# kentril0/WaterSurfaceRendering

Measured on AMD Instinct MI355X. Metric: ocean frames/s (ComputeWaves, 7 fields -> displacement + normal map), higher is better.
Workload: dtype f32; 1 GPU; 2048x2048 tile, FULL7, reference default parameters; tile_size=2048, tiles_per_rank=1, pipeline_depth=3, seed=1592590336, parallelism=tiles sharded 1 process per GPU x1, no data-path collective

## Files before the change

watersurfacerendering_amd/csrc/ocean_kernels.h:

```cpp
#pragma once
#include <hip/hip_runtime.h>
#include <hip/hip_fp16.h>
#include <stdint.h>
#include <type_traits>
#include "fft_engine.h"

namespace ocean {

typedef float ocean_f4 __attribute__((ext_vector_type(4)));
__device__ __forceinline__ void store_nt(float4* p, float4 v)
{
    ocean_f4 t = {v.x, v.y, v.z, v.w};
    __builtin_nontemporal_store(t, reinterpret_cast<ocean_f4*>(p));
}
__device__ __forceinline__ void store_f2_sc1(float2* base, unsigned byte_off, float2 v)
{
    typedef float f2v __attribute__((ext_vector_type(2)));
    const f2v t = {v.x, v.y};
    asm volatile("global_store_dwordx2 %0, %1, %2 sc1" ::"v"(byte_off), "v"(t), "s"(base) : "memory");
}
template <bool NTS> __device__ __forceinline__ void store_map(float4* base, unsigned texel, float4 v)
{
    float4* p = reinterpret_cast<float4*>(reinterpret_cast<char*>(base) + (texel * 16u));
    if constexpr (NTS) store_nt(p, v);
// ... 227 lines not shown
            float4 ha[PB];
            float2 hb0[PB], hb1[PB], wv[PB];
#pragma unroll
            for (int u = 0; u < PB; ++u) {
                const int it = tid + (ub + u) * T;
                const int c = COLS == 1 ? 0 : it / PAIRS, n = 2 * (COLS == 1 ? it : it % PAIRS);
                if (!GUARD || it < ITEMS) zpass_load_pair<N, H16, W16, ZNT>(a, tile, nb + c, n, h16s, base, ha[u], hb0[u], hb1[u], wv[u]);
            }
#pragma unroll
            for (int u = 0; u < PB; ++u) {
                const int it = tid + (ub + u) * T;
                const int c = COLS == 1 ? 0 : it / PAIRS, n = 2 * (COLS == 1 ? it : it % PAIRS);
                if (!GUARD || it < ITEMS) {
                    float a0, b0, a1, b1;
                    animate_with_mirror(make_float2(ha[u].x, ha[u].y), hb0[u], wv[u].x, t, a0, b0);
                    animate_with_mirror(make_float2(ha[u].z, ha[u].w), hb1[u], wv[u].y, t, a1, b1);
                    *reinterpret_cast<float2*>((c ? sp + N : sp) + n) = col0 ? make_float2(a0, a1) : make_float2(0.5f * (a0 + b0), 0.5f * (a1 + b1));
                    if constexpr (KZ_LDS) *reinterpret_cast<float2*>(kzt + n) = *reinterpret_cast<const float2*>(k1 + n);
                    if (n == 0) raw[c] = 0.5f * (a0 - b0);
                }
            }
        }
    });
}

template <int N> struct Half {
    static constexpr int NU = N / 2 + 1;
    static constexpr int NUP = (N / 2 + 16) & ~15;
    static constexpr size_t Z_GROUP = (size_t)NU * 2 * NUP;
    static constexpr size_t Z_TILE = 3 * Z_GROUP;
    static constexpr size_t ZH_TILE = (size_t)NU * NUP;
    static constexpr size_t HRAW_TILE = (size_t)NUP * N;
    template <bool Z16> static constexpr int zb() { return Z16 ? 16 : 8; }
    static_assert(NUP % 16 == 0, "row blocks");
    template <bool Z16> static __device__ __forceinline__ unsigned zidx(int nb, int side, int q)
    {
        constexpr int ZB = zb<Z16>();
        return (unsigned)(((q / ZB) * 2 + side) * (NU * ZB) + nb * ZB + (q % ZB));
    }
    template <bool Z16> static __device__ __forceinline__ unsigned zhidx(int nb, int q)
    {
        constexpr int ZB = zb<Z16>() > 8 ? zb<Z16>() : 8;
        return (unsigned)((q / ZB) * (NU * ZB) + nb * ZB + (q % ZB));
    }
};
__device__ __forceinline__ unsigned hraw_index(int n, int p, int u) { return (unsigned)(u * n + p); }

__device__ __forceinline__ int xcd_swizzle(int id, int n)
{
    const int q = n / 8, r = n % 8, x = id % 8;
    return (x < r ? x * (q + 1) : r * (q + 1) + (x - r) * q) + id / 8;
}

template <int N, int T, class P, int ZC, bool Z16> struct ZStore {
    using HF = Half<N>;
    using LS = LastStage<N, ZC, T, P>;
    static constexpr int S = LS::STRIDE, NU = HF::NU;
    static constexpr int ZB = HF::template zb<Z16>(), ZBH = ZB > 8 ? ZB : 8;
    static constexpr bool FAST = S >= ZBH && S % ZBH == 0 && (N / 2) % S == 0 && !(Z16 && ZC == 4);
    int b0[LS::IT], b1[LS::IT], bh[LS::IT];
    static __device__ __forceinline__ int reg(int v) { asm("" : "+v"(v)); return v; }
    __device__ __forceinline__ void init(int tid, int nb, bool two_columns = false)
    {
        if constexpr (FAST) {
#pragma unroll
            for (int u = 0; u < LS::IT; ++u) {
                const int w = tid + u * T;
                int c = 0, j = 0;
                if (!LS::GUARD || w < LS::ITEMS) LS::map(w, c, j);
                const int col = nb + (two_columns ? c : 0);
                b0[u] = (j / ZB) * (2 * NU * ZB) + (j % ZB) + col * ZB;
                const int cj = (j + ZB - 1) / ZB, rj = (ZB - j % ZB) % ZB;
                b1[u] = NU * ZB + col * ZB + rj - cj * (2 * NU * ZB);
                bh[u] = (j / ZBH) * (NU * ZBH) + (j % ZBH) + col * ZBH;
            }
        }
    }
    __device__ __forceinline__ unsigned pos(int col, int p, int u, int i) const
    {
        if constexpr (!FAST) return p <= N / 2 ? HF::template zidx<Z16>(col, 0, p) : HF::template zidx<Z16>(col, 1, N - p);
        else {
            const int lo = i * S;
            if (lo < N / 2) return (unsigned)(reg(b0[u]) + (lo / ZB) * (2 * NU * ZB));
            const int far = reg(b1[u]) + ((N - lo) / ZB) * (2 * NU * ZB);
            if (lo > N / 2) return (unsigned)far;
            return (unsigned)(far - (p == N / 2 ? NU * ZB : 0));
        }
    }
    __device__ __forceinline__ bool keeps(int p, int i) const
    {
        if constexpr (!FAST) return p <= N / 2;
        else return i * S < N / 2 || (i * S == N / 2 && p == N / 2);
    }
    __device__ __forceinline__ unsigned hpos(int col, int p, int u, int i) const
    {
        if constexpr (!FAST) return HF::template zhidx<Z16>(col, p);
        else return (unsigned)(reg(bh[u]) + ((i * S) / ZBH) * (NU * ZBH));
    }
};


template <int N> constexpr int zpass_columns() { return (N == 512 || N == 256) ? 4 : 2; }
template <int N> constexpr bool zpass_has_width2() { return zpass_columns<N>() == 2 && N >= 1024 && N <= 2048; }

template <int FIRST, int SLOTS>
__device__ __forceinline__ c32 zpass_input_slot(int c, float kx, float kx2, float kz, float sv, float tx, float tz, float tc,
                                                float choppy, float full7, bool jac, float g3)
{
#pragma clang fp contract(off)
    static_assert(FIRST + SLOTS <= 4 && (SLOTS == 1 || SLOTS == 4 || (SLOTS == 2 && FIRST % 2 == 0)), "one pair, {pair 0, pair 1}, {pair 2, pair 3} or all four");
    constexpr bool ODD_PAIRS = FIRST < 2, EVEN_PAIRS = FIRST + SLOTS > 2;
    const int pair = SLOTS == 1 ? FIRST : FIRST + c;
    const float d = __builtin_fmaf(kz, kz, kx2);
    const float inv = d > 1e-10f ? rsqrtf(d) : 0.0f;
    if (ODD_PAIRS && (!EVEN_PAIRS || pair < 2)) {
        const float f = (pair ? -1.0f : inv) * choppy;
        return make_float2(kz * f * tz, -kx * f * tx);
    }
    const float g = full7 * inv * sv;
    return pair == 2 ? make_float2(kx2 * g, kz * kz * g) : make_float2(sv, jac ? g3 * (kx * kz * inv * tc) : 0.0f);
}
template <int PAIR>
__device__ __forceinline__ c32 zpass_input(float kx, float kx2, float kz, float sv, float tx, float tz, float tc, bool jac, float g3)
{
#pragma clang fp contract(off)
    const float d = __builtin_fmaf(kz, kz, kx2);
    const float inv = d > 1e-10f ? rsqrtf(d) : 0.0f;
    if constexpr (PAIR == 0) { const float f = inv; return make_float2(kz * f * tz, -kx * f * tx); }
    else if constexpr (PAIR == 1) { const float f = -1.0f; return make_float2(kz * f * tz, -kx * f * tx); }
    else if constexpr (PAIR == 2) { const float g = inv * sv; return make_float2(kx2 * g, (kz * kz) * g); }
    else return make_float2(sv, jac ? g3 * (kx * kz * inv * tc) : 0.0f);
}
template <int N, bool COL0>
__device__ __forceinline__ void zpass_fetch(const float* sp, float sm0, int e, float& sv, float& tx, float& tz, float& tc)
{
    if constexpr (COL0) {
        const float g1 = sp[e], g2 = sp[(N - e) & (N - 1)];
        sv = 0.5f * (g1 + g2);
        tx = 0.5f * (g1 - g2);
        tz = (e == 0) ? tx : sv;
        tc = (e == 0) ? sv : tx;
    } else {
        sv = sp[e];
        tx = sv;
        tz = (e == 0) ? sm0 : sv;
        tc = tz;
    }
}
template <int N, bool Z16> struct ZOut {
    float su = 1.0f, sk = 1.0f, s3 = 1.0f, g3 = 1.0f;
    float2* __restrict__ zt;
    float2* __restrict__ z3;
// ... 156 lines not shown
        }
        if (blk == LAST) { one_column(N / 2); return; }
        one_column(0);
        __syncthreads();
        one_column(1);
    } else {
        one_column(xcd_swizzle(bx, gx));
    }
}

template <int N, int T, class P = Plan<N>, bool ZNT = false, bool Z16 = false, int ZW = 1, bool FAST = true>
__global__ void __launch_bounds__(T, zpass_min_waves<N>()) k_zpass(const FrameArgs a)
{
    extern __shared__ __attribute__((aligned(16))) unsigned char smem[];
    zpass_body<N, T, P, ZNT, Z16, ZW, FAST>(a, smem, (int)blockIdx.x, (int)gridDim.x);
}

__device__ __forceinline__ void start_ramp_wait(int ramp, unsigned idx, unsigned count)
{
    if (ramp > 0) {
        const unsigned until = idx * (unsigned)ramp / count;
        const unsigned long long t0 = wall_clock64();
        while ((unsigned)(wall_clock64() - t0) < until) __builtin_amdgcn_s_sleep(4);
    }
}

#ifdef OCEAN_CLOCKPROBE
static __device__ unsigned long long* g_clockprobe = nullptr;
constexpr unsigned CLOCKPROBE_LAUNCHES = 4096, CLOCKPROBE_WGS = 1032;
struct ClockProbe {
    unsigned long long* p;
    unsigned long long c0, r0;
    __device__ explicit ClockProbe(unsigned launch) : p(nullptr), c0(0), r0(0)
    {
        if (threadIdx.x == 0 && g_clockprobe && blockIdx.y == 0 && blockIdx.x < CLOCKPROBE_WGS) {
            p = g_clockprobe + 4 * ((size_t)(launch % CLOCKPROBE_LAUNCHES) * CLOCKPROBE_WGS + blockIdx.x);
            c0 = __builtin_amdgcn_s_memtime();
            r0 = __builtin_amdgcn_s_memrealtime();
        }
    }
    __device__ void end()
    {
        if (p) {
            const unsigned long long c1 = __builtin_amdgcn_s_memtime(), r1 = __builtin_amdgcn_s_memrealtime();
            unsigned hwid, xcc;
            asm volatile("s_getreg_b32 %0, hwreg(HW_REG_HW_ID)" : "=s"(hwid));
            asm volatile("s_getreg_b32 %0, hwreg(HW_REG_XCC_ID)" : "=s"(xcc));
            p[0] = r0; p[1] = r1; p[2] = c1 - c0; p[3] = (unsigned long long)xcc | ((unsigned long long)hwid << 32);
        }
    }
};
#endif

template <int N, int T, class P, bool COL0, bool ZNT, bool Z16, bool ZWT = false>
__device__ __forceinline__ void zpass_single_transforms(const FrameArgs& a, c32* fbuf, const float* sp, const float (&kzr)[P::r[0]],
                                                        TwiddleRegs<N, 1, T, P>& twr, float kx, float sm0, int tid, int tile, int nb)
{
    using HF = Half<N>;
    static_assert(FirstStage<N, 1, T, P>::IT == 1, "one first-stage butterfly per thread");
    const float kx2 = kx * kx;
    [[maybe_unused]] float su = 1.0f, sk = 1.0f, s3 = 1.0f;
    float g3 = 1.0f;
    if constexpr (Z16) { const float4 zs = a.zscale[2 * tile]; su = zs.x; sk = zs.y; s3 = a.zscale[2 * tile + 1].x; }
    if (a.mode == 3) g3 = a.zscale[2 * tile + 1].y;
    constexpr size_t ES = Z16 ? 4 : 8;
    float2* __restrict__ zt = reinterpret_cast<float2*>(reinterpret_cast<char*>(a.z) + (size_t)tile * HF::Z_TILE * ES);
    float2* __restrict__ z3 = reinterpret_cast<float2*>(reinterpret_cast<char*>(a.z3) + (size_t)tile * HF::Z_GROUP * ES);
    float2* __restrict__ zh = reinterpret_cast<float2*>(reinterpret_cast<char*>(a.zh) + (size_t)tile * HF::ZH_TILE * ES);
    const bool jac = a.mode == 3;
    ZStore<N, T, P, 1, Z16> zo;
    zo.init(tid, nb);
    auto fetch = [&](int e, float& sv, float& tx, float& tz, float& tc) {
        if constexpr (COL0) {
            const float g1 = sp[e], g2 = sp[(N - e) & (N - 1)];
            sv = 0.5f * (g1 + g2);
            tx = 0.5f * (g1 - g2);
            tz = (e == 0) ? tx : sv;
            tc = (e == 0) ? sv : tx;
        } else {
            sv = sp[e];
            tx = sv;
            tz = (e == 0) ? sm0 : sv;
            tc = tz;
        }
    };
    if (a.mode != 2) {
        if (a.zmask & 1) {
            auto in = [&](int e, int, int, int i) -> c32 {
                float sv, tx, tz, tc; fetch(e, sv, tx, tz, tc);
                return zpass_input<0>(kx, kx2, kzr[i], sv, tx, tz, tc, false, 1.0f);
            };
            auto out = [&](int p, int, c32 v, int u, int i) { store_z<ZNT, Z16, ZWT>(zt, zo.pos(nb, p, u, i), v, su); };
            batch_fft<N, 1, T, P>(fbuf, twr, tid, in, out);
        }
        if (a.zmask & 2) {
            auto in = [&](int e, int, int, int i) -> c32 {
                float sv, tx, tz, tc; fetch(e, sv, tx, tz, tc);
                return zpass_input<1>(kx, kx2, kzr[i], sv, tx, tz, tc, false, 1.0f);
            };
            auto out = [&](int p, int, c32 v, int u, int i) { store_z<ZNT, Z16, ZWT>(zt, (unsigned)HF::Z_GROUP + zo.pos(nb, p, u, i), v, sk); };
            batch_fft<N, 1, T, P>(fbuf, twr, tid, in, out);
        }
    }
    if ((a.mode == 0 || a.mode == 3) && (a.zmask & 4)) {
        auto in = [&](int e, int, int, int i) -> c32 {
            float sv, tx, tz, tc; fetch(e, sv, tx, tz, tc);
            return zpass_input<2>(kx, kx2, kzr[i], sv, tx, tz, tc, false, 1.0f);
        };
        auto out = [&](int p, int, c32 v, int u, int i) { store_z<ZNT, Z16, ZWT>(zt, 2u * (unsigned)HF::Z_GROUP + zo.pos(nb, p, u, i), v, sk); };
        batch_fft<N, 1, T, P>(fbuf, twr, tid, in, out);
    }
    if (a.zmask & 8) {
        auto in = [&](int e, int, int, int i) -> c32 {
            float sv, tx, tz, tc; fetch(e, sv, tx, tz, tc);
            if (!jac) return make_float2(sv, 0.0f);
            return zpass_input<3>(kx, kx2, kzr[i], sv, tx, tz, tc, true, g3);
        };
        auto out = [&](int p, int, c32 v, int u, int i) {
            if (jac) store_z<ZNT, Z16, ZWT>(z3, zo.pos(nb, p, u, i), v, s3);
            else if (zo.keeps(p, i)) store_z<ZNT, Z16, ZWT>(zh, zo.hpos(nb, p, u, i), v, su);
        };
        batch_fft<N, 1, T, P>(fbuf, twr, tid, in, out);
    }
}

template <int N> constexpr size_t zpass_c1_lds_bytes() { return sizeof(c32) * fft_lds_elems<N, 1>() + sizeof(float) * N; }
template <int N, int T, bool FAST> constexpr int zpass_c1_min_waves() { return T == N / 16 ? 3 : (FAST ? 6 : 5); }
template <int N, int T, class P, bool ZNT = false, bool Z16 = false, bool FAST = true, bool ZWT = false>
__global__ void __launch_bounds__(T, (zpass_c1_min_waves<N, T, FAST>())) k_zpass_c1(const FrameArgs a)
{
    extern __shared__ __attribute__((aligned(16))) unsigned char smem[];
    c32* fbuf = reinterpret_cast<c32*>(smem);
    float* sp = reinterpret_cast<float*>(fbuf + fft_lds_elems<N, 1>());
    float* raw = reinterpret_cast<float*>(fbuf);
    const int tid = threadIdx.x;
    const int tile = blockIdx.y;
#ifdef OCEAN_CLOCKPROBE
    ClockProbe clock_probe_(a.frame_seq);
#endif
    start_ramp_wait(a.start_ramp, blockIdx.x, gridDim.x);
    TwiddleRegs<N, 1, T, P> twr;
    twr.load(a.tw, tid);
#ifdef OCEAN_DEVELOPER
    const int bxr = (blockIdx.x % 8 == 0 || a.xcd_rot == 0) ? (int)blockIdx.x : (int)(blockIdx.x / 8 * 8 + 1 + (blockIdx.x % 8 - 1 + a.xcd_rot) % 7);
    const int nb = xcd_swizzle(bxr, N / 2 + 1);
#else
    const int nb = xcd_swizzle((int)blockIdx.x, N / 2 + 1);
#endif
    const float t = a.t + (a.toff ? a.toff[tile] : 0.0f);
    const float* __restrict__ k1 = a.k1d + (size_t)tile * N;
    const bool col0 = (nb == 0);
    const float h16s = a.h0h ? a.h0_inv_scale[tile] : 1.0f;
    const float base = a.omega_q ? a.base_freq[tile] : 0.0f;
    spectrum_form<FAST>(a, [&](auto h16, auto w16) {
        constexpr bool H16 = decltype(h16)::value, W16 = decltype(w16)::value;
        constexpr int PAIRS = N / 2;
        constexpr int P1 = (PAIRS + T - 1) / T;
        constexpr int PB = P1 > 4 ? 4 : P1;
        static_assert(P1 % PB == 0 && PAIRS % T == 0, "phase-1 batches");
#pragma unroll 1
        for (int ub = 0; ub < P1; ub += PB) {
            float4 ha[PB];
            float2 hb0[PB], hb1[PB], wv[PB];
#pragma unroll
            for (int u = 0; u < PB; ++u)
                zpass_load_pair<N, H16, W16, ZNT>(a, tile, nb, 2 * (tid + (ub + u) * T), h16s, base, ha[u], hb0[u], hb1[u], wv[u]);
#pragma unroll
            for (int u = 0; u < PB; ++u) {
                const int n = 2 * (tid + (ub + u) * T);
                float a0, b0, a1, b1;
                animate_with_mirror(make_float2(ha[u].x, ha[u].y), hb0[u], wv[u].x, t, a0, b0);
                animate_with_mirror(make_float2(ha[u].z, ha[u].w), hb1[u], wv[u].y, t, a1, b1);
                *reinterpret_cast<float2*>(sp + n) = col0 ? make_float2(a0, a1) : make_float2(0.5f * (a0 + b0), 0.5f * (a1 + b1));
                if (n == 0) raw[0] = 0.5f * (a0 - b0);
            }
        }
    });
    if (blockIdx.x == 0 && tid == 0 && (a.zmask & 8)) {
        a.minmax[2 * tile + 0] = float_key(3.402823466e+38f);
        a.minmax[2 * tile + 1] = float_key(1.175494351e-38f);
        a.hdone[tile] = 0u;
    }
    float kzr[P::r[0]];
#pragma unroll
    for (int i = 0; i < P::r[0]; ++i) kzr[i] = k1[tid + i * (N / P::r[0])];
    __syncthreads();
    const float sm0 = raw[0];
    static_assert(!ZWT || (!ZNT && !Z16), "write-through is a policy of the plain fp32 intermediates");
    if (col0) zpass_single_transforms<N, T, P, true, ZNT, Z16, ZWT>(a, fbuf, sp, kzr, twr, k1[nb], sm0, tid, tile, nb);
    else zpass_single_transforms<N, T, P, false, ZNT, Z16, ZWT>(a, fbuf, sp, kzr, twr, k1[nb], sm0, tid, tile, nb);
#ifdef OCEAN_CLOCKPROBE
    clock_probe_.end();
#endif
}
template <int N> constexpr bool zpass_has_c1() { return N >= 1024; }
template <int N> inline bool zpass_c1_pays(bool nt_inter, unsigned tiles)
{
    if (N == 4096) return true;
    if (nt_inter) return false;
    return N == 2048 || tiles >= 2;
}

template <int N, int T> constexpr int zpass_blocks_per_cu()
{
    constexpr int by_lds = (int)(163840 / (sizeof(c32) * fft_lds_elems<N, zpass_columns<N>()>() + sizeof(float) * 2 * N));
    constexpr int by_threads = 2048 / T;
    constexpr int by_regs = (zpass_min_waves<N>() * 4 * 64) / T;
    constexpr int m = by_lds < by_threads ? by_lds : by_threads;
    return (by_regs >= 1 && by_regs < m) ? by_regs : (m < 1 ? 1 : m);
}

template <int N, int ZW = 1> constexpr size_t zpass_lds_bytes()
{
    return sizeof(c32) * fft_lds_elems<N, zpass_columns<N>()>() + sizeof(float) * 2 * N;
}


__device__ __forceinline__ void store_wt(float* p, float v) { __hip_atomic_store(p, v, __ATOMIC_RELAXED, __HIP_MEMORY_SCOPE_AGENT); }
__device__ __forceinline__ float load_wt(const float* p) { return __hip_atomic_load(p, __ATOMIC_RELAXED, __HIP_MEMORY_SCOPE_AGENT); }
__device__ __forceinline__ unsigned load_wt(const unsigned* p) { return __hip_atomic_load(p, __ATOMIC_RELAXED, __HIP_MEMORY_SCOPE_AGENT); }
__device__ __forceinline__ void wait_counter(const unsigned* ctr, unsigned target, int tid, int poll_sleep = 0, unsigned* fault = nullptr)
{
    if (tid == 0) {
#ifdef OCEAN_FAULT_INJECT
        target += 1u;
#endif
        const unsigned long long t0 = wall_clock64();
        bool ok;
        while (!(ok = load_wt(ctr) >= target) && (wall_clock64() - t0) < 2000000ull) {
            if (poll_sleep <= 0) __builtin_amdgcn_s_sleep(2);
            else for (int k = 0; k < poll_sleep; ++k) __builtin_amdgcn_s_sleep(127);
        }
        if (!ok && fault) *fault = 1u;
    }
    __syncthreads();
}

__device__ __forceinline__ void wait_counter_reached(const unsigned* ctr, unsigned target, int tid, int poll_sleep = 0, unsigned* fault = nullptr)
{
    if (tid == 0) {
        const unsigned long long t0 = wall_clock64();
        bool ok;
        while (!(ok = (int)(load_wt(ctr) - target) >= 0) && (wall_clock64() - t0) < 2000000ull) {
            if (poll_sleep <= 0) __builtin_amdgcn_s_sleep(2);
            else for (int k = 0; k < poll_sleep; ++k) __builtin_amdgcn_s_sleep(127);
        }
        if (!ok && fault) *fault = 1u;
    }
    __syncthreads();
}

template <int N, bool Z16 = false>
__device__ __forceinline__ c32 load_pair_column(const float2* __restrict__ zg, int mf, int u, float eps, float unscale = 1.0f, float unscale_y = 0.0f)
{
    using HF = Half<N>;
    if (mf <= N / 2) return load_z<Z16>(zg, HF::template zidx<Z16>(mf, 0, u), unscale, unscale_y);
    const int side = (u == 0 || u == N / 2) ? 0 : 1;
    if constexpr (Z16) return load_z<true>(zg, HF::template zidx<Z16>(N - mf, side, u), eps * unscale, eps * unscale_y);
    const c32 v = load_z<false>(zg, HF::template zidx<Z16>(N - mf, side, u), 1.0f);
    return make_float2(eps * v.x, eps * v.y);
}
template <bool Z16> __device__ __forceinline__ const float2* z_base(const float2* base, size_t elems) { return reinterpret_cast<const float2*>(reinterpret_cast<const char*>(base) + elems * (Z16 ? 4 : 8)); }
template <int N, bool Z16> __device__ __forceinline__ const float2* pair_base(const float2* z, int tile, int pair) { return z_base<Z16>(z, (size_t)tile * Half<N>::Z_TILE + (size_t)pair * Half<N>::Z_GROUP); }

template <class LS, int T, class F>
__device__ __forceinline__ void for_each_output(int tid, F f)
{
#pragma unroll
    for (int u = 0; u < LS::IT; ++u) {
        const int w = tid + u * T;
        if (!LS::GUARD || w < LS::ITEMS) {
            int c, j;
            LS::map(w, c, j);
#pragma unroll
            for (int i = 0; i < LS::RL; ++i) f(j + i * LS::STRIDE, c, u, i);
        }
    }
}

template <int N, int C, int T, class P, int LM, bool NTS = true> constexpr bool mirror_rotates()
{
    return NTS && LM == 1 && C > 1 && (N / P::last) % 64 == 0 && T % 64 == 0 && ((N / P::last) * C) % T == 0;
}
template <int N, int C, int T, class P> constexpr size_t mirror_handoff_bytes() { return mirror_rotates<N, C, T, P, 1>() ? sizeof(float4) * C * (N / 64) : 0; }
template <int N, int C> constexpr size_t xpass_red_offset() { return sizeof(c32) * fft_lds_elems<N, C>(); }
template <int T> constexpr size_t xpass_red_bytes() { return sizeof(float) * 2 * ((T + 63) / 64); }
template <int N, int C, int T> constexpr size_t mirror_handoff_offset() { return (xpass_red_offset<N, C>() + xpass_red_bytes<T>() + 15) / 16 * 16; }
template <int N, int C, int T, class P> constexpr size_t xpass_lds_bytes(bool reduces)
{
    constexpr size_t hand = mirror_handoff_bytes<N, C, T, P>();
    return hand ? mirror_handoff_offset<N, C, T>() + hand : xpass_red_offset<N, C>() + (reduces ? xpass_red_bytes<T>() : 0);
}
template <int N, int C, int T, class P> constexpr size_t xpass_b_lds_bytes() { return xpass_lds_bytes<N, C, T, P>(true); }
template <int N, int C, int T, class P> constexpr size_t xpass_disp_lds_bytes() { return xpass_lds_bytes<N, C, T, P>(false); }
template <int N, int C> __device__ __forceinline__ float* xpass_red(unsigned char* smem) { return reinterpret_cast<float*>(smem + xpass_red_offset<N, C>()); }
template <int N, int C, int T> __device__ __forceinline__ float4* mirror_handoff(unsigned char* smem) { return reinterpret_cast<float4*>(smem + mirror_handoff_offset<N, C, T>()); }
__device__ __forceinline__ float wave_next_lane(float v)
{
    return __builtin_bit_cast(float, __builtin_amdgcn_update_dpp(0, __builtin_bit_cast(int, v), 0x134, 0xf, 0xf, false));
}
template <int N, class LS, int T, class V>
__device__ __forceinline__ void publish_row_heads(float4* hand, int tid, int u0, V value)
{
    for_each_output<LS, T>(tid, [&](int p, int c, int u, int i) {
        if ((tid & 63) == 0) hand[c * (N / 64) + (p >> 6)] = value(p, u0 + c, u, i);
    });
}
template <int N, class LS, int T, bool NTS, class V, class S, class M>
__device__ __forceinline__ void store_rows_whole(float4* __restrict__ map, float4* __restrict__ map_host, const float4* hand, int tid, int u0, V value, S side, M mirror)
{
    __syncthreads();
    for_each_output<LS, T>(tid, [&](int p, int c, int u, int i) {
        const int q = u0 + c;
        const float4 o = value(p, q, u, i);
        float4 nx = make_float4(wave_next_lane(o.x), wave_next_lane(o.y), wave_next_lane(o.z), wave_next_lane(o.w));
        if ((tid & 63) == 63) nx = hand[c * (N / 64) + (((p >> 6) + 1) & (N / 64 - 1))];
        if (q > N / 2) return;
        side(p, q, o);
        store_map<NTS>(map, (unsigned)(q * N + p), o);
        store_map_host(map_host, (unsigned)(q * N + p), o);
        if (q == 0 || q == N / 2) return;
        const unsigned t = (unsigned)((N - q) * N + (N - 1 - p));
        const float4 m = mirror(nx);
        store_map<NTS>(map, t, m);
        store_map_host(map_host, t, m);
    });
}
template <int A, int B> __device__ __forceinline__ void launder(c32 (&x)[A][B])
{
#pragma unroll
    for (int u = 0; u < A; ++u)
#pragma unroll
        for (int i = 0; i < B; ++i) asm volatile("" : "+v"(x[u][i].x), "+v"(x[u][i].y));
}
struct mirror_nrm { __device__ __forceinline__ float4 operator()(float4 o) const { return make_float4(-o.x, -o.y, o.z, o.w); } };
struct mirror_disp { __device__ __forceinline__ float4 operator()(float4 o) const { return make_float4(-o.x, o.y, -o.z, o.w); } };
template <int N, bool NTS, class M>
__device__ __forceinline__ void store_texel_and_mirror(float4* map, float4* map_host, int p, int q, float4 o, M mirror)
{
    store_map<NTS>(map, (unsigned)(q * N + p), o);
    store_map_host(map_host, (unsigned)(q * N + p), o);
    if (q == 0 || q == N / 2) return;
    const unsigned t = (unsigned)((N - q) * N + ((N - p) & (N - 1)));
    const float4 m = mirror(o);
    store_map<NTS>(map, t, m);
    store_map_host(map_host, t, m);
}

template <int N, int C> constexpr bool xpass_single_row_group() { return C > 1 && N >= 1024 && (N / 2) % (2 * C) == 0; }
template <int N, int C> constexpr int xpass_height_groups() { return (N / 2 + 1 + 2 * C - 1) / (2 * C); }
template <int N, int C> constexpr int xpass_row_groups() { return (Half<N>::NU + C - 1) / C; }
template <int N, int C> constexpr int xpass_merged_groups() { return xpass_height_groups<N, C>() + 2 * xpass_row_groups<N, C>(); }

// ... 461 lines not shown
```

watersurfacerendering_amd/csrc/ocean_launch.h:

```cpp
#pragma once
#include <cstdlib>

#include "ocean_ctx.h"

using namespace ocean;

template <class K>
static hipError_t allow_lds(K kernel, size_t bytes)
{
    if (bytes <= 48 * 1024) return hipSuccess;
    return hipFuncSetAttribute(reinterpret_cast<const void*>(kernel), hipFuncAttributeMaxDynamicSharedMemorySize,
                               (int)bytes);
}

template <class K, class... A>
static void launch(K kernel, dim3 grid, dim3 block, size_t lds, hipStream_t st, hipEvent_t* ev, A... args)
{
    if (ev) hipExtLaunchKernelGGL(kernel, grid, block, (uint32_t)lds, st, ev[0], ev[1], 0, args...);
    else hipLaunchKernelGGL(kernel, grid, block, lds, st, args...);
}

template <int N> constexpr bool xmerge_pays(bool alone) { return alone ? N <= 128 : N <= 512; }

template <int N>
static hipError_t launch_frame(ocean_ctx* c, const FrameArgs& a, FrameLaunch& fl)
{
    const FramePolicy& p = fl.policy;
    const hipStream_t st = fl.stream;
    using G = Geo<N>;
    using HF = Half<N>;
    const unsigned tiles = c->tiles;
    hipError_t e;
    constexpr int C = G::CC;
    constexpr size_t lds_rows = zpass_lds_bytes<N, 1>();
    constexpr bool HAS2 = zpass_has_width2<N>();
    constexpr size_t lds_rows2 = zpass_lds_bytes<N, 2>();
    constexpr size_t lds_m = xpass_disp_lds_bytes<N, C, G::T_C, typename G::PC>(), lds_b = xpass_b_lds_bytes<N, C, G::T_C, typename G::PC>();
    static_assert(lds_b <= 80 * 1024, "two x-pass workgroups per compute unit");
    static_assert(HF::NUP % (2 * C) == 0, "height row blocks");
    constexpr unsigned hb_b = xpass_height_groups<N, C>(), nb = xpass_row_groups<N, C>(), xg = xpass_merged_groups<N, C>();
    const bool fast = !a.h0h && a.omega_q;
    const bool alone = p.alone;
    const unsigned cus = (unsigned)(c->cu_count > 0 ? c->cu_count : 0);
    int ramp_z = 0, ramp_b = 0, ramp_d = 0;
#ifdef OCEAN_DEVELOPER
    constexpr bool DEV = true;
#else
    constexpr bool DEV = false;
#endif
    constexpr bool HAS1 = DEV || N <= 1024;
    constexpr bool HASC1 = zpass_has_c1<N>();
    constexpr bool HAS2_PLAIN = DEV && HAS2;
    if (c->attr_n != (uint32_t)N) {
#define OCEAN_ALLOW_Z(znt, z16, fast) \
        if constexpr (HAS1) if ((e = allow_lds(k_zpass<N, G::T_ROWS, typename G::PR, znt, z16, 1, fast>, lds_rows)) != hipSuccess) return e; \
        if constexpr (HAS2 && (znt || HAS2_PLAIN)) if ((e = allow_lds(k_zpass<N, G::T_ROWS, typename G::PR, znt, z16, 2, fast>, lds_rows2)) != hipSuccess) return e; \
        if constexpr (HASC1) if ((e = allow_lds(k_zpass_c1<N, zpass_c1_threads<N>(), typename C1Plan<N>::type, znt, z16, fast>, zpass_c1_lds_bytes<N>())) != hipSuccess) return e; \
        if constexpr (HASC1 && zpass_has_wt<N>() && !znt && !z16) if ((e = allow_lds(k_zpass_c1<N, zpass_c1_threads<N>(), typename C1Plan<N>::type, false, false, fast, true>, zpass_c1_lds_bytes<N>())) != hipSuccess) return e;
#define OCEAN_ALLOW_Z2(fast) OCEAN_ALLOW_Z(false, false, fast) OCEAN_ALLOW_Z(true, false, fast) OCEAN_ALLOW_Z(false, true, fast) OCEAN_ALLOW_Z(true, true, fast)
        OCEAN_ALLOW_Z2(true) OCEAN_ALLOW_Z2(false)
#undef OCEAN_ALLOW_Z2
#undef OCEAN_ALLOW_Z
#define OCEAN_ALLOW_X1(kern, lds, z16, jac) \
        if ((e = allow_lds(kern<N, C, G::T_C, typename G::PC, false, z16, jac>, lds)) != hipSuccess) return e; \
        if ((e = allow_lds(kern<N, C, G::T_C, typename G::PC, true, z16, jac>, lds)) != hipSuccess) return e;
#define OCEAN_ALLOW_X2(kern, lds, jac) OCEAN_ALLOW_X1(kern, lds, false, jac) OCEAN_ALLOW_X1(kern, lds, true, jac)
#define OCEAN_ALLOW_X(kern, lds) OCEAN_ALLOW_X2(kern, lds, false) OCEAN_ALLOW_X2(kern, lds, true)
        OCEAN_ALLOW_X(k_xpass_b, lds_b)
        OCEAN_ALLOW_X(k_xpass_disp, lds_m)
#undef OCEAN_ALLOW_X
#undef OCEAN_ALLOW_X2
#undef OCEAN_ALLOW_X1
        c->attr_n = (uint32_t)N;
    }
    if (c->start_ramp && cus) {
        if (c->occ_n != N) {
            int oz = 0, oza = 0, ob = 0, od = 0;
            if constexpr (zpass_has_c1<N>()) {
                (void)hipOccupancyMaxActiveBlocksPerMultiprocessor(&oz, k_zpass_c1<N, zpass_c1_threads<N>(), typename C1Plan<N>::type, false, false, true>,
                                                                   zpass_c1_threads<N>(), zpass_c1_lds_bytes<N>());
                (void)hipOccupancyMaxActiveBlocksPerMultiprocessor(&oza, k_zpass_c1<N, zpass_c1_threads<N>(), typename C1Plan<N>::type, false, false, false>,
                                                                   zpass_c1_threads<N>(), zpass_c1_lds_bytes<N>());
            }
            (void)hipOccupancyMaxActiveBlocksPerMultiprocessor(&ob, k_xpass_b<N, C, G::T_C, typename G::PC, false, false, false>, G::T_C, lds_b);
            (void)hipOccupancyMaxActiveBlocksPerMultiprocessor(&od, k_xpass_disp<N, C, G::T_C, typename G::PC, false, false, false>, G::T_C, lds_m);
            (void)hipGetLastError();
            c->occ_z = oz; c->occ_z_all = oza; c->occ_b = ob; c->occ_d = od; c->occ_n = N;
        }
        int bpt[3];
        ocean_launch_bytes_per_texel(p.half_inter, a.mode == 3, a.h0h != nullptr, a.omega_q != nullptr, bpt);
        const OceanTuning& tu = c->tune;
        const double texels = (double)tiles * N * N;
        auto ramp_ticks = [&](int bytes_per_texel, unsigned workgroups, int per_cu, double scale) -> int {
            const double bytes = texels * bytes_per_texel;
            const unsigned slots = (unsigned)per_cu < tu.ramp_max_wg_per_cu ? (unsigned)per_cu : tu.ramp_max_wg_per_cu;
            if (per_cu <= 0 || workgroups > slots * cus || texels < tu.ramp_min_texels) return 0;
            return (int)(tu.ramp_frac * scale * bytes / tu.ramp_rate_bytes_per_s * 1.0e8 + 0.5);
        };
        ramp_z = ramp_ticks(bpt[0], (unsigned)(N / 2 + 1) * tiles, fast ? c->occ_z : c->occ_z_all, 1.0);
        ramp_b = ramp_ticks(bpt[1] - 4, (hb_b + nb) * tiles, c->occ_b, alone ? 1.0 : tu.ramp_pipelined_x);
        ramp_d = ramp_ticks(bpt[2], nb * tiles, c->occ_d, alone ? 1.0 : tu.ramp_pipelined_x);
    }
    bool c1 = HASC1 && zpass_c1_pays<N>(p.nt_inter, tiles);
    bool zw2 = HAS2 && !c1 && p.nt_inter;
    constexpr bool HAS_WT = HASC1 && zpass_has_wt<N>();
    const bool wt_frame = HAS_WT && alone && !p.nt_inter && !p.half_inter && c->z_write_through;
    bool z_wt = c1 && wt_frame;
    bool merged_x = xmerge_pays<N>(alone) && tiles == 1 && a.mode != 3 && c->merged_x &&
                    xg <= c->tune.handoff_wg_per_cu * cus;
    constexpr bool HAS_ONE = (N <= 128 || (DEV && N <= 512)) && G::T_ROWS == G::T_C;
    bool one_launch = HAS_ONE && !alone && tiles == 1 && a.mode <= 2 && fast && p.nt_normal && p.nt_disp && !p.nt_inter && !p.half_inter && c->merged_x &&
                      ((unsigned)(N / 2 + 1) + xg) <= c->tune.handoff_wg_per_cu * cus;
    int poll_sleep = (merged_x && !one_launch && !alone) ? 1 : 0;
#ifdef OCEAN_DEVELOPER
    {   static const char* const c1_env = getenv("OCEAN_ZC1");
        if (c1_env && HASC1) c1 = atoi(c1_env) != 0;
        zw2 = HAS2 && !c1 && p.nt_inter;
        static const char* const zw_env = getenv("OCEAN_ZW");
        if (zw_env && HAS2 && !c1) zw2 = atoi(zw_env) == 2;
        const char* const wt_env = getenv("OCEAN_Z_WT");
        z_wt = c1 && wt_frame && !(wt_env && atoi(wt_env) == 0);
        const char* const xm = getenv("OCEAN_XMERGE");
        if (xm) merged_x = atoi(xm) != 0 && a.mode != 3;
        const char* const ol = getenv("OCEAN_ONE_LAUNCH");
        if (ol) one_launch = one_launch && atoi(ol) != 0;
        const char* const ps = getenv("OCEAN_POLL_SLEEP");
        poll_sleep = ps ? atoi(ps) : (merged_x && !one_launch && !alone) ? 1 : 0;
        static const char* const rz = getenv("OCEAN_RAMP_Z"); static const char* const rb = getenv("OCEAN_RAMP_B"); static const char* const rd = getenv("OCEAN_RAMP_D");
        static const char* const ra = getenv("OCEAN_RAMP_ANY");
        const bool on = ramp_z || ramp_b || ramp_d || (ra && atoi(ra) == 1);
        if (rz && on) ramp_z = atoi(rz);
        if (rb && on) ramp_b = atoi(rb);
        if (rd && on) ramp_d = atoi(rd); }
#endif
    fl.handoff = merged_x || one_launch;
    fl.launch_count = 0;
    auto next_marks = [&](int kernel) -> hipEvent_t* {
        const int l = fl.launch_count++;
        fl.launch_kernel[l] = kernel;
        return fl.marks ? fl.marks + 2 * l : nullptr;
    };
    auto describe = [&](int idx, unsigned grid_x, unsigned block, unsigned per_workgroup, size_t lds, uint32_t flags) {
        ocean_launch_info& li = c->last_launch[idx];
        li.tile_size = N; li.grid_x = grid_x; li.grid_y = tiles; li.block = block; li.mode = (uint32_t)a.mode;
        li.per_workgroup = per_workgroup;
        li.lds_bytes = (uint32_t)lds;
        li.flags = flags | (p.half_inter ? OCEAN_LAUNCH_HALF_INTER : 0u) | (a.mode == 3 ? OCEAN_LAUNCH_JACOBIAN : 0u);
    };
    const int rec_last = a.rec_mode;
    auto launch_z = [&]() -> hipError_t {
        const unsigned gx = zw2 ? N / 4 + 1 : N / 2 + 1;
        FrameArgs za = a;
        za.rec_mode = 0;
        za.start_ramp = c1 ? ramp_z : 0;
        const unsigned threads = c1 ? (unsigned)zpass_c1_threads<N>() : (unsigned)G::T_ROWS;
        const size_t lds = c1 ? zpass_c1_lds_bytes<N>() : (zw2 ? lds_rows2 : lds_rows);
        const dim3 grid(gx, tiles), block(threads);
        describe(0, gx, threads, zw2 ? 2u : 1u, lds,
                 (p.nt_inter ? OCEAN_LAUNCH_NT_INTER : 0u) | (a.h0h ? OCEAN_LAUNCH_FP16_SPECTRUM : 0u) |
                 (a.omega_q ? 0u : OCEAN_LAUNCH_FP32_DISPERSION) | (c1 ? OCEAN_LAUNCH_SINGLE_TRANSFORM : 0u) |
                 (za.start_ramp ? OCEAN_LAUNCH_STAGGERED_START : 0u) | (z_wt ? OCEAN_LAUNCH_WT_INTER : 0u));
        hipEvent_t* mz = next_marks(0);
#ifdef OCEAN_CLOCKPROBE
        {
            static unsigned long long* armed = nullptr;
            if (armed != c->stamps) { armed = c->stamps; (void)hipMemcpyToSymbol(HIP_SYMBOL(ocean::g_clockprobe), &armed, sizeof(armed)); }
        }
#endif
        bool launched = false;
        if constexpr (HAS_WT) {
            if (z_wt) {
                if (fast) launch(k_zpass_c1<N, zpass_c1_threads<N>(), typename C1Plan<N>::type, false, false, true, true>, grid, block, lds, st, mz, za);
                else launch(k_zpass_c1<N, zpass_c1_threads<N>(), typename C1Plan<N>::type, false, false, false, true>, grid, block, lds, st, mz, za);
                launched = true;
            }
        }
#define OCEAN_ZPASS3(znt, z16, fast) \
        do { if (launched) break; if constexpr (HASC1) { if (c1) { launch(k_zpass_c1<N, zpass_c1_threads<N>(), typename C1Plan<N>::type, znt, z16, fast>, grid, block, lds, st, mz, za); launched = true; break; } } \
             if constexpr (HAS2 && (znt || HAS2_PLAIN)) { if (zw2) { launch(k_zpass<N, G::T_ROWS, typename G::PR, znt, z16, 2, fast>, grid, block, lds, st, mz, za); launched = true; break; } } \
             if constexpr (HAS1) { if (!c1 && !zw2) { launch(k_zpass<N, G::T_ROWS, typename G::PR, znt, z16, 1, fast>, grid, block, lds, st, mz, za); launched = true; } } } while (0)
#define OCEAN_ZPASS2(znt, z16) \
        do { if (fast) OCEAN_ZPASS3(znt, z16, true); else OCEAN_ZPASS3(znt, z16, false); } while (0)
#define OCEAN_ZPASS(znt) \
        do { if (p.half_inter) OCEAN_ZPASS2(znt, true); else OCEAN_ZPASS2(znt, false); } while (0)
        if (p.nt_inter) OCEAN_ZPASS(true); else OCEAN_ZPASS(false);
#undef OCEAN_ZPASS
#undef OCEAN_ZPASS2
#undef OCEAN_ZPASS3
        if (!launched) return hipErrorInvalidConfiguration;
        return hipSuccess;
    };
    const bool jac = a.mode == 3;
    const unsigned hb = jac ? nb : hb_b;
    const dim3 blk(G::T_C);
#define OCEAN_XPASS2(kern, grid, lds, ev, nts, z16, args)                                                          \
        do { if (jac) launch(kern<N, C, G::T_C, typename G::PC, nts, z16, true>, grid, blk, lds, st, ev, args);       \
             else launch(kern<N, C, G::T_C, typename G::PC, nts, z16, false>, grid, blk, lds, st, ev, args); } while (0)
#define OCEAN_XPASS(kern, grid, lds, ev, nts, args)                                                                 \
        do { if (p.half_inter) OCEAN_XPASS2(kern, grid, lds, ev, nts, true, args);                                  \
             else OCEAN_XPASS2(kern, grid, lds, ev, nts, false, args); } while (0)
    auto launch_xb = [&](bool merged) {
        const dim3 gb(hb + nb + (merged ? nb : 0u), tiles);
        const uint32_t flags_b = (ramp_b ? OCEAN_LAUNCH_STAGGERED_START : 0u) | (merged ? OCEAN_LAUNCH_MERGED_X : 0u);
        describe(1, gb.x, G::T_C, C, lds_b, flags_b | (p.nt_normal ? OCEAN_LAUNCH_NT_MAPS : 0u));
        if (merged) describe(2, gb.x, G::T_C, C, lds_b, flags_b | (p.nt_disp ? OCEAN_LAUNCH_NT_MAPS : 0u));
        hipEvent_t* mb = next_marks(1);
        FrameArgs ba = a;
        ba.xb_disp = merged ? 1 : 0; ba.rec_mode = merged ? rec_last : 0;
        ba.poll_sleep = poll_sleep;
        ba.start_ramp = ramp_b;
        if (p.nt_normal) OCEAN_XPASS(k_xpass_b, gb, lds_b, mb, true, ba);
        else OCEAN_XPASS(k_xpass_b, gb, lds_b, mb, false, ba);
    };
    auto launch_xd = [&]() {
        const dim3 gd(nb, tiles);
        describe(2, gd.x, G::T_C, C, lds_m, (p.nt_disp ? OCEAN_LAUNCH_NT_MAPS : 0u) | (ramp_d ? OCEAN_LAUNCH_STAGGERED_START : 0u));
        hipEvent_t* md = next_marks(2);
        FrameArgs da = a;
        da.rec_mode = rec_last;
        da.start_ramp = ramp_d;
        if (p.nt_disp) OCEAN_XPASS(k_xpass_disp, gd, lds_m, md, true, da);
        else OCEAN_XPASS(k_xpass_disp, gd, lds_m, md, false, da);
    };
    if constexpr (HAS_ONE) {
// ... 34 lines not shown
```

Measured before the change: 21980 frames/s.

## Store side-1 z outputs as whole rotated pieces via lane shuffle in pipelined 2048 frames

Adds a rotated store path for the single-transform z pass. Side-1 (mirrored) outputs are shifted by one element using a DPP next-lane shuffle plus a small LDS handoff for run boundaries, so each wave writes contiguous aligned pieces instead of misaligned mirrored addresses. It also turns on the write-through intermediate path for the pipelined (depth 3, single tile) N=2048 case, which uses the new kernel variant. The cost is extra LDS, a barrier, and holding the second-half outputs in registers, which may raise register pressure.

```diff
diff --git a/watersurfacerendering_amd/csrc/ocean_kernels.h b/watersurfacerendering_amd/csrc/ocean_kernels.h
--- a/watersurfacerendering_amd/csrc/ocean_kernels.h
+++ b/watersurfacerendering_amd/csrc/ocean_kernels.h
@@ -303,12 +303,13 @@
     return (x < r ? x * (q + 1) : r * (q + 1) + (x - r) * q) + id / 8;
 }
 
-template <int N, int T, class P, int ZC, bool Z16> struct ZStore {
+template <int N, int T, class P, int ZC, bool Z16, bool ROT = false> struct ZStore {
     using HF = Half<N>;
     using LS = LastStage<N, ZC, T, P>;
     static constexpr int S = LS::STRIDE, NU = HF::NU;
     static constexpr int ZB = HF::template zb<Z16>(), ZBH = ZB > 8 ? ZB : 8;
     static constexpr bool FAST = S >= ZBH && S % ZBH == 0 && (N / 2) % S == 0 && !(Z16 && ZC == 4);
+    static_assert(!ROT || FAST, "the rotated side-1 stores build on the per-item bases");
     int b0[LS::IT], b1[LS::IT], bh[LS::IT];
     static __device__ __forceinline__ int reg(int v) { asm("" : "+v"(v)); return v; }
     __device__ __forceinline__ void init(int tid, int nb, bool two_columns = false)
@@ -321,7 +322,8 @@
                 if (!LS::GUARD || w < LS::ITEMS) LS::map(w, c, j);
                 const int col = nb + (two_columns ? c : 0);
                 b0[u] = (j / ZB) * (2 * NU * ZB) + (j % ZB) + col * ZB;
-                const int cj = (j + ZB - 1) / ZB, rj = (ZB - j % ZB) % ZB;
+                const int j1 = ROT ? j + 1 : j;
+                const int cj = (j1 + ZB - 1) / ZB, rj = (ZB - j1 % ZB) % ZB;
                 b1[u] = NU * ZB + col * ZB + rj - cj * (2 * NU * ZB);
                 bh[u] = (j / ZBH) * (NU * ZBH) + (j % ZBH) + col * ZBH;
             }
@@ -329,6 +331,7 @@
     }
     __device__ __forceinline__ unsigned pos(int col, int p, int u, int i) const
     {
+        static_assert(!ROT, "the rotated forms address by pos0 / pos1_next");
         if constexpr (!FAST) return p <= N / 2 ? HF::template zidx<Z16>(col, 0, p) : HF::template zidx<Z16>(col, 1, N - p);
         else {
             const int lo = i * S;
@@ -348,7 +351,58 @@
         if constexpr (!FAST) return HF::template zhidx<Z16>(col, p);
         else return (unsigned)(reg(bh[u]) + ((i * S) / ZBH) * (NU * ZBH));
     }
+    __device__ __forceinline__ unsigned pos0(int u, int i) const { return (unsigned)(reg(b0[u]) + ((i * S) / ZB) * (2 * NU * ZB)); }
+    __device__ __forceinline__ unsigned pos1_next(int u, int i) const { return (unsigned)(reg(b1[u]) + ((N - i * S) / ZB) * (2 * NU * ZB)); }
 };
+
+template <int N, int T, class P, int ZC, bool Z16> constexpr bool zpass_rotates(bool past_l2)
+{
+    using LS = LastStage<N, ZC, T, P>;
+    return past_l2 && (ZC == 1 || ZC == 2) && ZStore<N, T, P, ZC, Z16>::FAST && !LS::GUARD && T % 64 == 0 && LS::ITEMS % 64 == 0 &&
+           LS::STRIDE % (64 / ZC) == 0 && (N / 2) % LS::STRIDE == 0;
+}
+template <int N, int ZC> constexpr size_t zpass_handoff_bytes() { return sizeof(float2) * ZC * ((N / 2) / (64 / ZC)); }
+__device__ __forceinline__ float wave_next_lane(float v)
+{
+    return __builtin_bit_cast(float, __builtin_amdgcn_update_dpp(0, __builtin_bit_cast(int, v), 0x134, 0xf, 0xf, false));
+}
+template <int N, int ZC, int T, class P, class In, class Low, class High>
+__device__ __forceinline__ void zpass_batch_whole(c32* fbuf, TwiddleRegs<N, ZC, T, P>& twr, int tid, c32* hand, bool side1, In& in, Low&& low, High&& high)
+{
+    using LS = LastStage<N, ZC, T, P>;
+    constexpr int S = LS::STRIDE, FIRST = (N / 2) / S, LEGS = LS::RL - FIRST, RUN = 64 / ZC, RUNS = (N / 2) / RUN;
+    c32 held[LS::IT][LEGS];
+    auto out = [&](int p, int, c32 v, int u, int i) {
+        if (i < FIRST) { low(u, i, v); return; }
+        held[u][i - FIRST] = v;
+        if (i == FIRST && p == N / 2) low(u, i, v);
+    };
+    batch_fft<N, ZC, T, P>(fbuf, twr, tid, in, out);
+    if (!side1) return;
+    const bool first = (tid & (RUN - 1)) == 0, last = (tid & (RUN - 1)) == RUN - 1;
+#pragma unroll
+    for (int u = 0; u < LS::IT; ++u) {
+        int c, j;
+        LS::map(tid + u * T, c, j);
+        if (first) {
+#pragma unroll
+            for (int l = 0; l < LEGS; ++l) hand[c * RUNS + (j + l * S) / RUN] = held[u][l];
+        }
+    }
+    __syncthreads();
+#pragma unroll
+    for (int u = 0; u < LS::IT; ++u) {
+        int c, j;
+        LS::map(tid + u * T, c, j);
+#pragma unroll
+        for (int l = 0; l < LEGS; ++l) {
+            const int pn = j + l * S + 1;
+            c32 nx = make_float2(wave_next_lane(held[u][l].x), wave_next_lane(held[u][l].y));
+            if (last && pn < N / 2) nx = hand[c * RUNS + pn / RUN];
+            if (pn < N / 2) high(u, FIRST + l, nx);
+        }
+    }
+}
 
 
 template <int N> constexpr int zpass_columns() { return (N == 512 || N == 256) ? 4 : 2; }
@@ -611,9 +665,9 @@
 };
 #endif
 
-template <int N, int T, class P, bool COL0, bool ZNT, bool Z16, bool ZWT = false>
+template <int N, int T, class P, bool COL0, bool ZNT, bool Z16, bool ZWT = false, bool ZROT = false>
 __device__ __forceinline__ void zpass_single_transforms(const FrameArgs& a, c32* fbuf, const float* sp, const float (&kzr)[P::r[0]],
-                                                        TwiddleRegs<N, 1, T, P>& twr, float kx, float sm0, int tid, int tile, int nb)
+                                                        TwiddleRegs<N, 1, T, P>& twr, float kx, float sm0, int tid, int tile, int nb, c32* hand)
 {
     using HF = Half<N>;
     static_assert(FirstStage<N, 1, T, P>::IT == 1, "one first-stage butterfly per thread");
@@ -627,8 +681,15 @@
     float2* __restrict__ z3 = reinterpret_cast<float2*>(reinterpret_cast<char*>(a.z3) + (size_t)tile * HF::Z_GROUP * ES);
     float2* __restrict__ zh = reinterpret_cast<float2*>(reinterpret_cast<char*>(a.zh) + (size_t)tile * HF::ZH_TILE * ES);
     const bool jac = a.mode == 3;
-    ZStore<N, T, P, 1, Z16> zo;
+    static_assert(!ZROT || ZWT, "whole pieces from side 1: a form of the write-through stores");
+    constexpr bool ROT = ZROT && zpass_rotates<N, T, P, 1, Z16>(ZWT);
+    ZStore<N, T, P, 1, Z16, ROT> zo;
     zo.init(tid, nb);
+    [[maybe_unused]] auto whole = [&](auto& in, float2* base, unsigned group, float scale) {
+        zpass_batch_whole<N, 1, T, P>(fbuf, twr, tid, hand, true, in,
+                                      [&](int u, int i, c32 v) { store_z<ZNT, Z16, ZWT>(base, group + zo.pos0(u, i), v, scale); },
+                                      [&](int u, int i, c32 v) { store_z<ZNT, Z16, ZWT>(base, group + zo.pos1_next(u, i), v, scale); });
+    };
     auto fetch = [&](int e, float& sv, float& tx, float& tz, float& tc) {
         if constexpr (COL0) {
             const float g1 = sp[e], g2 = sp[(N - e) & (N - 1)];
@@ -649,16 +710,22 @@
                 float sv, tx, tz, tc; fetch(e, sv, tx, tz, tc);
                 return zpass_input<0>(kx, kx2, kzr[i], sv, tx, tz, tc, false, 1.0f);
             };
-            auto out = [&](int p, int, c32 v, int u, int i) { store_z<ZNT, Z16, ZWT>(zt, zo.pos(nb, p, u, i), v, su); };
-            batch_fft<N, 1, T, P>(fbuf, twr, tid, in, out);
+            if constexpr (ROT) whole(in, zt, 0u, su);
+            else {
+                auto out = [&](int p, int, c32 v, int u, int i) { store_z<ZNT, Z16, ZWT>(zt, zo.pos(nb, p, u, i), v, su); };
+                batch_fft<N, 1, T, P>(fbuf, twr, tid, in, out);
+            }
         }
         if (a.zmask & 2) {
             auto in = [&](int e, int, int, int i) -> c32 {
                 float sv, tx, tz, tc; fetch(e, sv, tx, tz, tc);
                 return zpass_input<1>(kx, kx2, kzr[i], sv, tx, tz, tc, false, 1.0f);
             };
-            auto out = [&](int p, int, c32 v, int u, int i) { store_z<ZNT, Z16, ZWT>(zt, (unsigned)HF::Z_GROUP + zo.pos(nb, p, u, i), v, sk); };
-            batch_fft<N, 1, T, P>(fbuf, twr, tid, in, out);
+            if constexpr (ROT) whole(in, zt, (unsigned)HF::Z_GROUP, sk);
+            else {
+                auto out = [&](int p, int, c32 v, int u, int i) { store_z<ZNT, Z16, ZWT>(zt, (unsigned)HF::Z_GROUP + zo.pos(nb, p, u, i), v, sk); };
+                batch_fft<N, 1, T, P>(fbuf, twr, tid, in, out);
+            }
         }
     }
     if ((a.mode == 0 || a.mode == 3) && (a.zmask & 4)) {
@@ -666,8 +733,11 @@
             float sv, tx, tz, tc; fetch(e, sv, tx, tz, tc);
             return zpass_input<2>(kx, kx2, kzr[i], sv, tx, tz, tc, false, 1.0f);
         };
-        auto out = [&](int p, int, c32 v, int u, int i) { store_z<ZNT, Z16, ZWT>(zt, 2u * (unsigned)HF::Z_GROUP + zo.pos(nb, p, u, i), v, sk); };
-        batch_fft<N, 1, T, P>(fbuf, twr, tid, in, out);
+        if constexpr (ROT) whole(in, zt, 2u * (unsigned)HF::Z_GROUP, sk);
+        else {
+            auto out = [&](int p, int, c32 v, int u, int i) { store_z<ZNT, Z16, ZWT>(zt, 2u * (unsigned)HF::Z_GROUP + zo.pos(nb, p, u, i), v, sk); };
+            batch_fft<N, 1, T, P>(fbuf, twr, tid, in, out);
+        }
     }
     if (a.zmask & 8) {
         auto in = [&](int e, int, int, int i) -> c32 {
@@ -675,23 +745,33 @@
             if (!jac) return make_float2(sv, 0.0f);
             return zpass_input<3>(kx, kx2, kzr[i], sv, tx, tz, tc, true, g3);
         };
-        auto out = [&](int p, int, c32 v, int u, int i) {
-            if (jac) store_z<ZNT, Z16, ZWT>(z3, zo.pos(nb, p, u, i), v, s3);
-            else if (zo.keeps(p, i)) store_z<ZNT, Z16, ZWT>(zh, zo.hpos(nb, p, u, i), v, su);
-        };
-        batch_fft<N, 1, T, P>(fbuf, twr, tid, in, out);
-    }
-}
-
-template <int N> constexpr size_t zpass_c1_lds_bytes() { return sizeof(c32) * fft_lds_elems<N, 1>() + sizeof(float) * N; }
+        if constexpr (ROT) {
+            zpass_batch_whole<N, 1, T, P>(fbuf, twr, tid, hand, jac, in,
+                                          [&](int u, int i, c32 v) {
+                                              if (jac) store_z<ZNT, Z16, ZWT>(z3, zo.pos0(u, i), v, s3);
+                                              else store_z<ZNT, Z16, ZWT>(zh, zo.hpos(nb, 0, u, i), v, su);
+                                          },
+                                          [&](int u, int i, c32 v) { store_z<ZNT, Z16, ZWT>(z3, zo.pos1_next(u, i), v, s3); });
+        } else {
+            auto out = [&](int p, int, c32 v, int u, int i) {
+                if (jac) store_z<ZNT, Z16, ZWT>(z3, zo.pos(nb, p, u, i), v, s3);
+                else if (zo.keeps(p, i)) store_z<ZNT, Z16, ZWT>(zh, zo.hpos(nb, p, u, i), v, su);
+            };
+            batch_fft<N, 1, T, P>(fbuf, twr, tid, in, out);
+        }
+    }
+}
+
+template <int N> constexpr size_t zpass_c1_lds_bytes() { return sizeof(c32) * fft_lds_elems<N, 1>() + sizeof(float) * N + zpass_handoff_bytes<N, 1>(); }
 template <int N, int T, bool FAST> constexpr int zpass_c1_min_waves() { return T == N / 16 ? 3 : (FAST ? 6 : 5); }
-template <int N, int T, class P, bool ZNT = false, bool Z16 = false, bool FAST = true, bool ZWT = false>
+template <int N, int T, class P, bool ZNT = false, bool Z16 = false, bool FAST = true, bool ZWT = false, bool ZROT = false>
 __global__ void __launch_bounds__(T, (zpass_c1_min_waves<N, T, FAST>())) k_zpass_c1(const FrameArgs a)
 {
     extern __shared__ __attribute__((aligned(16))) unsigned char smem[];
     c32* fbuf = reinterpret_cast<c32*>(smem);
     float* sp = reinterpret_cast<float*>(fbuf + fft_lds_elems<N, 1>());
     float* raw = reinterpret_cast<float*>(fbuf);
+    c32* hand = reinterpret_cast<c32*>(sp + N);
     const int tid = threadIdx.x;
     const int tile = blockIdx.y;
 #ifdef OCEAN_CLOCKPROBE
@@ -746,8 +826,8 @@
     __syncthreads();
     const float sm0 = raw[0];
     static_assert(!ZWT || (!ZNT && !Z16), "write-through is a policy of the plain fp32 intermediates");
-    if (col0) zpass_single_transforms<N, T, P, true, ZNT, Z16, ZWT>(a, fbuf, sp, kzr, twr, k1[nb], sm0, tid, tile, nb);
-    else zpass_single_transforms<N, T, P, false, ZNT, Z16, ZWT>(a, fbuf, sp, kzr, twr, k1[nb], sm0, tid, tile, nb);
+    if (col0) zpass_single_transforms<N, T, P, true, ZNT, Z16, ZWT, ZROT>(a, fbuf, sp, kzr, twr, k1[nb], sm0, tid, tile, nb, hand);
+    else zpass_single_transforms<N, T, P, false, ZNT, Z16, ZWT, ZROT>(a, fbuf, sp, kzr, twr, k1[nb], sm0, tid, tile, nb, hand);
 #ifdef OCEAN_CLOCKPROBE
     clock_probe_.end();
 #endif
@@ -854,10 +934,6 @@
 template <int N, int C, int T, class P> constexpr size_t xpass_disp_lds_bytes() { return xpass_lds_bytes<N, C, T, P>(false); }
 template <int N, int C> __device__ __forceinline__ float* xpass_red(unsigned char* smem) { return reinterpret_cast<float*>(smem + xpass_red_offset<N, C>()); }
 template <int N, int C, int T> __device__ __forceinline__ float4* mirror_handoff(unsigned char* smem) { return reinterpret_cast<float4*>(smem + mirror_handoff_offset<N, C, T>()); }
-__device__ __forceinline__ float wave_next_lane(float v)
-{
-    return __builtin_bit_cast(float, __builtin_amdgcn_update_dpp(0, __builtin_bit_cast(int, v), 0x134, 0xf, 0xf, false));
-}
 template <int N, class LS, int T, class V>
 __device__ __forceinline__ void publish_row_heads(float4* hand, int tid, int u0, V value)
 {
diff --git a/watersurfacerendering_amd/csrc/ocean_launch.h b/watersurfacerendering_amd/csrc/ocean_launch.h
--- a/watersurfacerendering_amd/csrc/ocean_launch.h
+++ b/watersurfacerendering_amd/csrc/ocean_launch.h
@@ -56,7 +56,8 @@
         if constexpr (HAS1) if ((e = allow_lds(k_zpass<N, G::T_ROWS, typename G::PR, znt, z16, 1, fast>, lds_rows)) != hipSuccess) return e; \
         if constexpr (HAS2 && (znt || HAS2_PLAIN)) if ((e = allow_lds(k_zpass<N, G::T_ROWS, typename G::PR, znt, z16, 2, fast>, lds_rows2)) != hipSuccess) return e; \
         if constexpr (HASC1) if ((e = allow_lds(k_zpass_c1<N, zpass_c1_threads<N>(), typename C1Plan<N>::type, znt, z16, fast>, zpass_c1_lds_bytes<N>())) != hipSuccess) return e; \
-        if constexpr (HASC1 && zpass_has_wt<N>() && !znt && !z16) if ((e = allow_lds(k_zpass_c1<N, zpass_c1_threads<N>(), typename C1Plan<N>::type, false, false, fast, true>, zpass_c1_lds_bytes<N>())) != hipSuccess) return e;
+        if constexpr (HASC1 && zpass_has_wt<N>() && !znt && !z16) if ((e = allow_lds(k_zpass_c1<N, zpass_c1_threads<N>(), typename C1Plan<N>::type, false, false, fast, true>, zpass_c1_lds_bytes<N>())) != hipSuccess) return e; \
+        if constexpr (HASC1 && N == 2048 && !znt && !z16) if ((e = allow_lds(k_zpass_c1<N, zpass_c1_threads<N>(), typename C1Plan<N>::type, false, false, fast, true, true>, zpass_c1_lds_bytes<N>())) != hipSuccess) return e;
 #define OCEAN_ALLOW_Z2(fast) OCEAN_ALLOW_Z(false, false, fast) OCEAN_ALLOW_Z(true, false, fast) OCEAN_ALLOW_Z(false, true, fast) OCEAN_ALLOW_Z(true, true, fast)
         OCEAN_ALLOW_Z2(true) OCEAN_ALLOW_Z2(false)
 #undef OCEAN_ALLOW_Z2
@@ -104,7 +105,8 @@
     bool c1 = HASC1 && zpass_c1_pays<N>(p.nt_inter, tiles);
     bool zw2 = HAS2 && !c1 && p.nt_inter;
     constexpr bool HAS_WT = HASC1 && zpass_has_wt<N>();
-    const bool wt_frame = HAS_WT && alone && !p.nt_inter && !p.half_inter && c->z_write_through;
+    const bool wt_pipelined = HAS_WT && N == 2048 && !alone && tiles == 1 && c->depth == 3;
+    const bool wt_frame = HAS_WT && (alone || wt_pipelined) && !p.nt_inter && !p.half_inter && c->z_write_through;
     bool z_wt = c1 && wt_frame;
     bool merged_x = xmerge_pays<N>(alone) && tiles == 1 && a.mode != 3 && c->merged_x &&
                     xg <= c->tune.handoff_wg_per_cu * cus;
@@ -169,7 +171,14 @@
 #endif
         bool launched = false;
         if constexpr (HAS_WT) {
-            if (z_wt) {
+            if constexpr (N == 2048) {
+                if (z_wt && !alone) {
+                    if (fast) launch(k_zpass_c1<N, zpass_c1_threads<N>(), typename C1Plan<N>::type, false, false, true, true, true>, grid, block, lds, st, mz, za);
+                    else launch(k_zpass_c1<N, zpass_c1_threads<N>(), typename C1Plan<N>::type, false, false, false, true, true>, grid, block, lds, st, mz, za);
+                    launched = true;
+                }
+            }
+            if (z_wt && !launched) {
                 if (fast) launch(k_zpass_c1<N, zpass_c1_threads<N>(), typename C1Plan<N>::type, false, false, true, true>, grid, block, lds, st, mz, za);
                 else launch(k_zpass_c1<N, zpass_c1_threads<N>(), typename C1Plan<N>::type, false, false, false, true>, grid, block, lds, st, mz, za);
                 launched = true;
```

After: 22670 frames/s, median of 4. +3.1%, better.
